# phymhan/supervised-gan

Hardware: AMD Instinct MI355X
Metric: train-step images/sec, fcgan 512x512 bs=1/GPU (higher is better)
Workload: dtype f32 (bf16x3 MFMA); 1 GPU; fcgan deconv-G(ngf32, z 8x8x8) + 3x PatchGAN-D(ndf32, n_layers 3, scale 1/2/4) 512x512 bs=1, n_update_D=1 n_update_G=2, Adam, pool 50 (BASELINE configs[1] shape, fp32 compute); synthetic batches resident in HBM (ring of 64); parallelism=dp1, global_batch=1, hip_graph=True, skip_wasted_D_wgrad=False

## Files before the change

### supervised-gan_amd/csrc/sgan_ew.hip

```cpp
#include "sgan_reduce.h"

thread_local char g_sgan_err[512] = {0};
thread_local const char* g_sgan_last_kernel = "";
thread_local char g_sgan_last_variant[96] = {0};

int sgan_fail(int code, const char* fmt, ...) {
    va_list ap;
    va_start(ap, fmt);
    vsnprintf(g_sgan_err, sizeof(g_sgan_err), fmt, ap);
    va_end(ap);
    return code;
}

extern "C" const char* sgan_version(void) { return "sgan_hip 0.2 (gfx950; fp32 MFMA 16x16x4 + split-bf16 MFMA 32x32x16)"; }
extern "C" const char* sgan_last_error(void) { return g_sgan_err; }
extern "C" const char* sgan_last_kernel(void) { return g_sgan_last_kernel; }
extern "C" const char* sgan_last_variant(void) { return g_sgan_last_variant; }
extern "C" int sgan_stat_replicas(void) { return SGAN_STAT_REPLICAS; }
extern "C" int sgan_set_device(int32_t device_id) {
    hipError_t e = hipSetDevice(device_id);
    if (e != hipSuccess) {
        (void)hipGetLastError();
        return sgan_fail(SGAN_ERR_HIP, "hipSetDevice(%d): %s", (int)device_id, hipGetErrorString(e));
    }
    return SGAN_OK;
}
extern "C" int sgan_stream_device(void* stream, int32_t* device_id) {
    if (!device_id) return sgan_fail(SGAN_ERR_INVALID, "null device_id");
    hipDevice_t dev;
    hipError_t e = hipStreamGetDevice((hipStream_t)stream, &dev);
    if (e != hipSuccess) {
        (void)hipGetLastError();
        return sgan_fail(SGAN_ERR_HIP, "hipStreamGetDevice: %s", hipGetErrorString(e));
    }
    *device_id = (int32_t)dev;
    return SGAN_OK;
}

#define SG_PROF_MAX 8192
static bool g_prof_on = false;
static int g_prof_n = 0;
static hipEvent_t g_prof_e0[SG_PROF_MAX], g_prof_e1[SG_PROF_MAX];
static const char* g_prof_name[SG_PROF_MAX];
static bool g_prof_open = false;

void sg_prof_begin(hipStream_t st) {
    if (!g_prof_on || g_prof_n >= SG_PROF_MAX) return;
    if (hipEventCreate(&g_prof_e0[g_prof_n]) != hipSuccess || hipEventCreate(&g_prof_e1[g_prof_n]) != hipSuccess) return;
    (void)hipEventRecord(g_prof_e0[g_prof_n], st);
    g_prof_open = true;
}

void sg_prof_end(hipStream_t st, const char* name) {
    if (!g_prof_open) return;
    (void)hipEventRecord(g_prof_e1[g_prof_n], st);
    g_prof_name[g_prof_n] = name;
    ++g_prof_n;
    g_prof_open = false;
}

extern "C" int sgan_profile_enable(int on) {
    for (int i = 0; i < g_prof_n; ++i) {
        (void)hipEventDestroy(g_prof_e0[i]);
        (void)hipEventDestroy(g_prof_e1[i]);
    }
    g_prof_n = 0;
    g_prof_on = on != 0;
    return SGAN_OK;
}

extern "C" int sgan_profile_count(void) { return g_prof_n; }

extern "C" int sgan_profile_mark(void* stream) {
    sg_prof_begin((hipStream_t)stream);
    sg_prof_end((hipStream_t)stream, "null");
    return SGAN_OK;
}

extern "C" int sgan_profile_read(int i, const char** name, float* ms) {
    if (i < 0 || i >= g_prof_n || !name || !ms) return sgan_fail(SGAN_ERR_INVALID, "bad profile record index");
    *name = g_prof_name[i];
    if (hipEventElapsedTime(ms, g_prof_e0[i], g_prof_e1[i]) != hipSuccess) return sgan_fail(SGAN_ERR_HIP, "hipEventElapsedTime failed");
    return SGAN_OK;
}

struct SgNormBwdJob {
    float* dy; const float* x; const double* sums; float* dgamma; float* dbeta; unsigned* amax;
    SgNorm xn;
    int32_t dy_ld, x_ld, npix, C, sums_sq, sums_rep, blocks;
};
struct SgNormBwdTable { SgNormBwdJob j[8]; };

__global__ __launch_bounds__(256) void sg_norm_bwd_apply_kernel(const SgNormBwdTable T) {
    sg_warm_kernargs<(int)sizeof(SgNormBwdTable)>();
    const SgNormBwdJob& J = T.j[blockIdx.y];
    if ((int)blockIdx.x >= J.blocks) return;
    const int C = J.C;
    extern __shared__ __attribute__((aligned(16))) char smem[];
    float* cA = reinterpret_cast<float*>(smem);
    float* cMean = cA + C;
    float* cRstd = cMean + C;
    float* cS1 = cRstd + C;
    float* cS2 = cS1 + C;
    const double invM = 1.0 / (double)J.npix;
    for (int c = threadIdx.x; c < C; c += 256) {
        float mean, rstd;
        sg_mean_rstd(J.xn, C, c, mean, rstd);
        const float g = J.xn.gamma ? J.xn.gamma[c] : 1.f;
        cA[c] = g * rstd;
        cMean[c] = mean;
        cRstd[c] = rstd;
        const double s1 = sg_stat_sum(J.sums, c, J.sums_rep), s2 = sg_stat_sum(J.sums, J.sums_sq + c, J.sums_rep);
        cS1[c] = (float)(s1 * invM);
        cS2[c] = (float)(s2 * invM);
        if (blockIdx.x == 0) {
            if (J.dgamma) atomicAdd(&J.dgamma[c], (float)s2);
            if (J.dbeta) atomicAdd(&J.dbeta[c], (float)s1);
        }
    }
    SG_SYNC();
    const int CQ = C >> 2;
    const int64_t total = (int64_t)J.npix * CQ;
    float* dy = J.dy;
    const float* x = J.x;
    const int64_t stride = (int64_t)J.blocks * 256;
    float amax = 0.f;
    for (int64_t e0 = (int64_t)blockIdx.x * 256 + threadIdx.x; e0 < total; e0 += 4 * stride) {
        f32x4 d[4], xv[4];
        int64_t od[4];
        int cc[4];
#pragma unroll
        for (int u = 0; u < 4; ++u) {
            const int64_t e = e0 + u * stride;
            const bool ok = e < total;
            const int p = ok ? (int)(e / CQ) : 0;
            cc[u] = ok ? (int)(e - (int64_t)p * CQ) * 4 : 0;
            od[u] = ok ? (int64_t)p * J.dy_ld + cc[u] : -1;
            d[u] = *reinterpret_cast<const f32x4*>(dy + (ok ? od[u] : 0));
            xv[u] = *reinterpret_cast<const f32x4*>(x + (ok ? (int64_t)p * J.x_ld + cc[u] : 0));
        }
#pragma unroll
        for (int u = 0; u < 4; ++u) {
            if (od[u] < 0) continue;
            const int c = cc[u];
#pragma unroll
            for (int j = 0; j < 4; ++j) {
                const float xhat = (xv[u][j] - cMean[c + j]) * cRstd[c + j];
                d[u][j] = cA[c + j] * (d[u][j] - cS1[c + j] - xhat * cS2[c + j]);
                amax = fmaxf(amax, fabsf(d[u][j]));
            }
            *reinterpret_cast<f32x4*>(dy + od[u]) = d[u];
        }
    }
    if (J.amax) {
        for (int o = 32; o > 0; o >>= 1) amax = fmaxf(amax, __shfl_xor(amax, o));
        SG_SYNC();
        if ((threadIdx.x & 63) == 0) cA[threadIdx.x >> 6] = amax;
        SG_SYNC();
        if (threadIdx.x == 0) {
            const unsigned mine = __builtin_bit_cast(unsigned, fmaxf(fmaxf(cA[0], cA[1]), fmaxf(cA[2], cA[3])));
            if (mine > __hip_atomic_load(J.amax, __ATOMIC_RELAXED, __HIP_MEMORY_SCOPE_AGENT)) atomicMax(J.amax, mine);
        }
    }
}

extern "C" int sgan_norm_bwd_apply_multi(const sgan_norm_bwd_job* jobs, int32_t n, void* stream) {
    SGAN_CHECK(jobs && n >= 1 && n <= 8, "1..8 jobs");
    SgNormBwdTable T;
    int maxb = 1, maxC = 4;
    for (int i = 0; i < n; ++i) {
        const sgan_norm_bwd_job& S = jobs[i];
        SGAN_CHECK(S.dy && S.x && S.x_norm && S.x_norm->stats && S.bwd_sums, "null argument in job %d", i);
        SGAN_CHECK((S.C & 3) == 0 && S.C > 0 && S.C <= 4096 && S.dy_ld >= S.C && S.x_ld >= S.C && (S.dy_ld & 3) == 0 &&
                       (S.x_ld & 3) == 0 && S.npix > 0, "bad dims in job %d", i);
        SgNormBwdJob& J = T.j[i];
        J.dy = S.dy; J.x = S.x; J.sums = S.bwd_sums; J.dgamma = S.dgamma; J.dbeta = S.dbeta;
        J.amax = reinterpret_cast<unsigned*>(S.amax_out);
        J.xn = sg_norm_from(S.x_norm);
        J.dy_ld = S.dy_ld; J.x_ld = S.x_ld; J.npix = S.npix; J.C = S.C;
        J.sums_sq = S.bwd_sums_sq_stride ? S.bwd_sums_sq_stride : S.C;
        J.sums_rep = S.bwd_sums_rep_stride;
        const int64_t total = (int64_t)S.npix * (S.C >> 2);
        static const int chunk = getenv("SGAN_NBA_CHUNK") ? atoi(getenv("SGAN_NBA_CHUNK")) : 4;
        int blocks = sg_cdiv(total, 256 * (chunk > 0 ? chunk : 4));
        if (blocks > 2048) blocks = 2048;
        if (blocks < 1) blocks = 1;
        J.blocks = blocks;
        if (blocks > maxb) maxb = blocks;
        if (S.C > maxC) maxC = S.C;
    }
    hipLaunchKernelGGL(sg_norm_bwd_apply_kernel, dim3(maxb, n), dim3(256), (size_t)5 * maxC * 4, (hipStream_t)stream, T);
    SGAN_LAUNCH_CHECK();
    g_sgan_last_kernel = "sg_norm_bwd_apply_kernel";
    return SGAN_OK;
}

extern "C" int sgan_norm_bwd_apply(float* dy, int32_t dy_ld, const float* x, int32_t x_ld, int32_t npix, int32_t C,
                                   const sgan_norm_desc* x_norm, const double* bwd_sums, int32_t bwd_sums_sq_stride,
                                   float* dgamma, float* dbeta, void* stream) {
    sgan_norm_bwd_job j = {dy, dy_ld, x, x_ld, npix, C, x_norm, bwd_sums, bwd_sums_sq_stride, dgamma, dbeta, 0, nullptr};
    return sgan_norm_bwd_apply_multi(&j, 1, stream);
}

__global__ __launch_bounds__(256) void sg_mean_rstd_probe_kernel(SgNorm n, int C, float* out) {
    for (int c = threadIdx.x; c < C; c += 256) {
        float mean, rstd;
        sg_mean_rstd(n, C, c, mean, rstd);
        out[2 * c] = mean;
        out[2 * c + 1] = rstd;
    }
}

extern "C" int sgan_norm_mean_rstd_probe(const sgan_norm_desc* d, int32_t C, float* out, void* stream) {
    SGAN_CHECK(d && d->stats && out && C > 0 && d->count > 0, "bad argument");
    hipLaunchKernelGGL(sg_mean_rstd_probe_kernel, dim3(1), dim3(256), 0, (hipStream_t)stream, sg_norm_from(d), C, out);
    SGAN_LAUNCH_CHECK();
    return SGAN_OK;
}

__global__ __launch_bounds__(256) void sg_norm_apply_fwd_kernel(const float* u, int u_ld, SgNorm un, const float* mask,
                                                                const float* noise, float sigma, float* t, int t_ld, int npix,
                                                                int C) {
    extern __shared__ __attribute__((aligned(16))) char smem[];
    float* cMean = reinterpret_cast<float*>(smem);
    float* cA = cMean + C;
    float* cB = cA + C;
    for (int c = threadIdx.x; c < C; c += 256) {
        float mean = 0.f, rstd = 1.f;
        if (un.stats) sg_mean_rstd(un, C, c, mean, rstd);
        cMean[c] = mean;
        cA[c] = (un.gamma ? un.gamma[c] : 1.f) * rstd;
        cB[c] = un.beta ? un.beta[c] : 0.f;
    }
    SG_SYNC();
    const int CQ = C >> 2;
    const int64_t total = (int64_t)npix * CQ;
    for (int64_t e = (int64_t)blockIdx.x * 256 + threadIdx.x; e < total; e += (int64_t)gridDim.x * 256) {
        const int p = (int)(e / CQ), c = (int)(e - (int64_t)p * CQ) * 4;
        const f32x4 x = *reinterpret_cast<const f32x4*>(u + (int64_t)p * u_ld + c);
        f32x4 m = (f32x4){1.f, 1.f, 1.f, 1.f}, nz = (f32x4){0.f, 0.f, 0.f, 0.f};
        if (mask) m = *reinterpret_cast<const f32x4*>(mask + (int64_t)p * C + c);
        if (noise) nz = *reinterpret_cast<const f32x4*>(noise + (int64_t)p * C + c);
        f32x4 o;
#pragma unroll
        for (int j = 0; j < 4; ++j) o[j] = ((x[j] - cMean[c + j]) * cA[c + j] + cB[c + j]) * m[j] + sigma * nz[j];
        *reinterpret_cast<f32x4*>(t + (int64_t)p * t_ld + c) = o;
    }
}

__global__ __launch_bounds__(256) void sg_norm_apply_bwd_sums_kernel(float* dt, int dt_ld, const float* mask, const float* u,
                                                                     int u_ld, SgNorm un, double* sums, int npix, int C) {
    extern __shared__ __attribute__((aligned(16))) char smem[];
    float* cMean = reinterpret_cast<float*>(smem);
    float* cRstd = cMean + C;
    float* red = cRstd + C;
    for (int c = threadIdx.x; c < C; c += 256) {
        float mean = 0.f, rstd = 1.f;
        if (un.stats) sg_mean_rstd(un, C, c, mean, rstd);
        cMean[c] = mean;
        cRstd[c] = rstd;
    }
    for (int i = threadIdx.x; i < 2 * C; i += 256) red[i] = 0.f;
    SG_SYNC();
    const int CQ = C >> 2;
    const int64_t total = (int64_t)npix * CQ;
    if (256 % CQ == 0) {
        const int c = (threadIdx.x % CQ) * 4;
        const f32x4 mean = *reinterpret_cast<const f32x4*>(cMean + c), rstd = *reinterpret_cast<const f32x4*>(cRstd + c);
        f32x4 s1 = (f32x4){0.f, 0.f, 0.f, 0.f}, s2 = s1;
        for (int64_t e = (int64_t)blockIdx.x * 256 + threadIdx.x; e < total; e += (int64_t)gridDim.x * 256) {
            const int64_t p = e / CQ;
            f32x4 d = *reinterpret_cast<const f32x4*>(dt + p * dt_ld + c);
            const f32x4 x = *reinterpret_cast<const f32x4*>(u + p * u_ld + c);
            if (mask) {
                d *= *reinterpret_cast<const f32x4*>(mask + p * C + c);
                *reinterpret_cast<f32x4*>(dt + p * dt_ld + c) = d;
            }
            s1 += d;
            s2 += d * ((x - mean) * rstd);
        }
#pragma unroll
        for (int j = 0; j < 4; ++j) {
            atomicAdd(&red[c + j], s1[j]);
            atomicAdd(&red[C + c + j], s2[j]);
        }
    } else {
        for (int64_t e = (int64_t)blockIdx.x * 256 + threadIdx.x; e < total; e += (int64_t)gridDim.x * 256) {
            const int p = (int)(e / CQ), c = (int)(e - (int64_t)p * CQ) * 4;
            f32x4 d = *reinterpret_cast<const f32x4*>(dt + (int64_t)p * dt_ld + c);
            const f32x4 x = *reinterpret_cast<const f32x4*>(u + (int64_t)p * u_ld + c);
            if (mask) {
                const f32x4 m = *reinterpret_cast<const f32x4*>(mask + (int64_t)p * C + c);
                d *= m;
                *reinterpret_cast<f32x4*>(dt + (int64_t)p * dt_ld + c) = d;
            }
#pragma unroll
            for (int j = 0; j < 4; ++j) {
                const float xhat = (x[j] - cMean[c + j]) * cRstd[c + j];
                atomicAdd(&red[c + j], d[j]);
                atomicAdd(&red[C + c + j], d[j] * xhat);
            }
        }
    }
    SG_SYNC();
    for (int c = threadIdx.x; c < C; c += 256) {
        atomicAdd(&sums[c], (double)red[c]);
        atomicAdd(&sums[C + c], (double)red[C + c]);
    }
}

extern "C" int sgan_norm_apply_fwd(const float* u, int32_t u_ld, const sgan_norm_desc* u_norm, const float* mask,
                                   const float* noise, float sigma, float* t, int32_t t_ld, int32_t npix, int32_t C, void* stream) {
    SGAN_CHECK(u && t && npix > 0 && C > 0 && (C & 3) == 0 && u_ld >= C && t_ld >= C && (u_ld & 3) == 0 && (t_ld & 3) == 0, "bad argument");
    const int64_t total = (int64_t)npix * (C >> 2);
    int blocks = sg_cdiv(total, 256 * 2);
    if (blocks > 2048) blocks = 2048;
    if (blocks < 1) blocks = 1;
    hipLaunchKernelGGL(sg_norm_apply_fwd_kernel, dim3(blocks), dim3(256), (size_t)3 * C * 4, (hipStream_t)stream, u, u_ld,
                       sg_norm_from(u_norm), mask, noise, sigma, t, t_ld, npix, C);
    SGAN_LAUNCH_CHECK();
    return SGAN_OK;
}

extern "C" int sgan_norm_apply_bwd_sums(float* dt, int32_t dt_ld, const float* mask, const float* u, int32_t u_ld,
                                        const sgan_norm_desc* u_norm, double* bwd_sums, int32_t npix, int32_t C, void* stream) {
    SGAN_CHECK(dt && u && bwd_sums && npix > 0 && C > 0 && (C & 3) == 0 && u_ld >= C && dt_ld >= C, "bad argument");
    const int64_t total = (int64_t)npix * (C >> 2);
    int blocks = sg_cdiv(total, 256 * 8);
    if (blocks > 512) blocks = 512;
    if (blocks < 1) blocks = 1;
    hipLaunchKernelGGL(sg_norm_apply_bwd_sums_kernel, dim3(blocks), dim3(256), (size_t)4 * C * 4, (hipStream_t)stream, dt, dt_ld,
                       mask, u, u_ld, sg_norm_from(u_norm), bwd_sums, npix, C);
    SGAN_LAUNCH_CHECK();
    return SGAN_OK;
}

__device__ __forceinline__ int sg_refl(int i, int n) { return i < 0 ? -i : (i >= n ? 2 * (n - 1) - i : i); }

__global__ __launch_bounds__(256) void sg_pad_reflect_fwd_kernel(const float* x, int x_ld, int H, int W, int C, SgNorm xn, const float* mask,
                                                                 int pad, float* out, int out_ld) {
    extern __shared__ __attribute__((aligned(16))) char smem[];
    float* cSc = reinterpret_cast<float*>(smem);
    float* cSh = cSc + C;
    for (int c = threadIdx.x; c < C; c += 256) {
        float sc = 1.f, sh = 0.f;
        if (xn.stats) {
            float mean, rstd;
            sg_mean_rstd(xn, C, c, mean, rstd);
            const float gm = xn.gamma ? xn.gamma[c] : 1.f, bt = xn.beta ? xn.beta[c] : 0.f;
            sc = gm * rstd;
            sh = bt - mean * sc;
        }
        cSc[c] = sc;
        cSh[c] = sh;
    }
    SG_SYNC();
    const int CQ = C >> 2, Wp = W + 2 * pad, Hp = H + 2 * pad;
    const int64_t total = (int64_t)Hp * Wp * CQ;
    for (int64_t e = (int64_t)blockIdx.x * 256 + threadIdx.x; e < total; e += (int64_t)gridDim.x * 256) {
        const int c = (int)(e % CQ) * 4;
        const int64_t pp = e / CQ;
        const int px = (int)(pp % Wp), py = (int)(pp / Wp);
        const int64_t src = (int64_t)sg_refl(py - pad, H) * W + sg_refl(px - pad, W);
        f32x4 v = *reinterpret_cast<const f32x4*>(x + src * x_ld + c);
#pragma unroll
        for (int j = 0; j < 4; ++j) v[j] = sg_act(v[j] * cSc[c + j] + cSh[c + j], xn.act, xn.slope);
        if (mask) v *= *reinterpret_cast<const f32x4*>(mask + src * C + c);
        *reinterpret_cast<f32x4*>(out + pp * out_ld + c) = v;
    }
}

extern "C" int sgan_pad_reflect_fwd(const float* x, int32_t x_ld, int32_t H, int32_t W, int32_t C, const sgan_norm_desc* x_norm,
                                    const float* mask, int32_t pad, float* out, int32_t out_ld, void* stream) {
    SGAN_CHECK(x && out && H > 0 && W > 0 && C > 0 && (C & 3) == 0 && (x_ld & 3) == 0 && (out_ld & 3) == 0 && x_ld >= C && out_ld >= C,
               "bad argument");
    SGAN_CHECK(pad >= 0 && pad < H && pad < W, "reflection padding must be smaller than the image");
    const int64_t total = (int64_t)(H + 2 * pad) * (W + 2 * pad) * (C >> 2);
    int blocks = sg_cdiv(total, 256 * 4);
    if (blocks > 2048) blocks = 2048;
    hipLaunchKernelGGL(sg_pad_reflect_fwd_kernel, dim3(blocks), dim3(256), (size_t)2 * C * 4, (hipStream_t)stream, x, x_ld, H, W, C,
                       sg_norm_from(x_norm), mask, pad, out, out_ld);
    SGAN_LAUNCH_CHECK();
    return SGAN_OK;
}

__global__ __launch_bounds__(256) void sg_pad_reflect_bwd_kernel(const float* dout, int dout_ld, int H, int W, int C, int pad, const float* x,
                                                                 int x_ld, SgNorm xn, const float* mask, float* din, int din_ld,
                                                                 double* sums, int sums_sq) {
    extern __shared__ __attribute__((aligned(16))) char smem[];
    float* cMean = reinterpret_cast<float*>(smem);
    float* cRstd = cMean + C;
    float* cG = cRstd + C;
    float* cB = cG + C;
    double* red = reinterpret_cast<double*>(cB + C);
    for (int c = threadIdx.x; c < C; c += 256) {
        float mean = 0.f, rstd = 1.f;
        if (xn.stats) sg_mean_rstd(xn, C, c, mean, rstd);
        cMean[c] = mean;
        cRstd[c] = rstd;
        cG[c] = (xn.stats && xn.gamma) ? xn.gamma[c] : 1.f;
        cB[c] = (xn.stats && xn.beta) ? xn.beta[c] : 0.f;
    }
    for (int i = threadIdx.x; i < 2 * C; i += 256) red[i] = 0.0;
    SG_SYNC();
    const int CQ = C >> 2, Wp = W + 2 * pad;
    const int64_t total = (int64_t)H * W * CQ;
    const bool has_x = x != nullptr;
    for (int64_t e = (int64_t)blockIdx.x * 256 + threadIdx.x; e < total; e += (int64_t)gridDim.x * 256) {
        const int c = (int)(e % CQ) * 4;
        const int64_t pix = e / CQ;
        const int xx = (int)(pix % W), yy = (int)(pix / W);
        int ys[3], xs[3], ny = 0, nx = 0;
        ys[ny++] = yy + pad;
        if (yy >= 1 && yy <= pad) ys[ny++] = pad - yy;
        if (yy <= H - 2 && yy >= H - 1 - pad) ys[ny++] = pad + 2 * (H - 1) - yy;
        xs[nx++] = xx + pad;
        if (xx >= 1 && xx <= pad) xs[nx++] = pad - xx;
        if (xx <= W - 2 && xx >= W - 1 - pad) xs[nx++] = pad + 2 * (W - 1) - xx;
        f32x4 d = (f32x4){0.f, 0.f, 0.f, 0.f};
        for (int a = 0; a < ny; ++a)
            for (int b = 0; b < nx; ++b) d += *reinterpret_cast<const f32x4*>(dout + ((int64_t)ys[a] * Wp + xs[b]) * dout_ld + c);
        if (mask) d *= *reinterpret_cast<const f32x4*>(mask + pix * C + c);
        if (has_x) {
            const f32x4 xv = *reinterpret_cast<const f32x4*>(x + pix * x_ld + c);
#pragma unroll
            for (int j = 0; j < 4; ++j) {
                const float xhat = (xv[j] - cMean[c + j]) * cRstd[c + j];
                const float y = xn.stats ? cG[c + j] * xhat + cB[c + j] : xv[j];
                d[j] *= sg_act_grad(y, xn.act, xn.slope);
                if (sums) {
                    atomicAdd(&red[c + j], (double)d[j]);
                    atomicAdd(&red[C + c + j], (double)(d[j] * xhat));
                }
            }
        }
        *reinterpret_cast<f32x4*>(din + pix * din_ld + c) = d;
    }
    if (sums) {
        SG_SYNC();
        for (int c = threadIdx.x; c < C; c += 256) {
            atomicAdd(&sums[c], red[c]);
            atomicAdd(&sums[(sums_sq ? sums_sq : C) + c], red[C + c]);
        }
    }
}

extern "C" int sgan_pad_reflect_bwd(const float* dout, int32_t dout_ld, int32_t H, int32_t W, int32_t C, int32_t pad, const float* x,
                                    int32_t x_ld, const sgan_norm_desc* x_norm, const float* mask, float* din, int32_t din_ld,
                                    double* bwd_sums, int32_t bwd_sums_sq_stride, void* stream) {
    SGAN_CHECK(dout && din && H > 0 && W > 0 && C > 0 && (C & 3) == 0 && (dout_ld & 3) == 0 && (din_ld & 3) == 0 && dout_ld >= C && din_ld >= C,
               "bad argument");
    SGAN_CHECK(pad >= 0 && 2 * pad < H && 2 * pad < W, "reflection padding must be smaller than half the image");
    SGAN_CHECK(!(bwd_sums && !x), "bwd_sums needs x");
    SGAN_CHECK(!x || ((x_ld & 3) == 0 && x_ld >= C), "bad x_ld");
    const int64_t total = (int64_t)H * W * (C >> 2);
    int blocks = sg_cdiv(total, 256 * 4);
    if (blocks > 1024) blocks = 1024;
    hipLaunchKernelGGL(sg_pad_reflect_bwd_kernel, dim3(blocks), dim3(256), (size_t)4 * C * 4 + (size_t)2 * C * 8, (hipStream_t)stream, dout,
                       dout_ld, H, W, C, pad, x, x_ld, sg_norm_from(x ? x_norm : nullptr), mask, din, din_ld, bwd_sums, bwd_sums_sq_stride);
    SGAN_LAUNCH_CHECK();
    return SGAN_OK;
}

#define SG_IMGLOSS_BLOCKS 256
__device__ __forceinline__ void sg_block_partial(double acc, double* part) {
    __shared__ double wsum[4];
    const double sum = sg_block_sum<4>(acc, wsum);
    if (threadIdx.x == 0) part[blockIdx.x] = sum;
}

__global__ __launch_bounds__(64) void sg_imgloss_fin_kernel(const double* part, int nparts, double scale, float* loss_out) {
    double acc = 0.0;
    for (int i = threadIdx.x; i < nparts; i += 64) acc += part[i];
    acc = sg_wave_sum(acc);
    if (threadIdx.x == 0) loss_out[0] = (float)(acc * scale);
}

__global__ __launch_bounds__(256) void sg_l1w_fwd_kernel(const float* x, int x_ld, const float* y, int y_ld, int npix, int C,
                                                         const float* a, int a_ld, const float* wts, int nw, float lambda,
                                                         double* part, float* g, int g_ld) {
    const double inv = 1.0 / ((double)npix * (double)C);
    double acc = 0.0;
    for (int p = blockIdx.x * 256 + threadIdx.x; p < npix; p += gridDim.x * 256) {
        float w = 1.f;
        if (a) {
            if (nw == 0) w = a[(int64_t)p * a_ld];
            for (int i = 0; i < nw; ++i) w += (a[(int64_t)p * a_ld + i] + 1.f) * 0.5f * (wts[i] - 1.f);
        }
        for (int c = 0; c < g_ld; ++c) {
            float gv = 0.f;
            if (c < C) {
                const float d = x[(int64_t)p * x_ld + c] - y[(int64_t)p * y_ld + c];
                acc += (double)(fabsf(d) * w);
                gv = (d > 0.f ? 1.f : (d < 0.f ? -1.f : 0.f)) * w * lambda * (float)inv;
// ... 1829 lines not shown
```

Before: 543.3 images/sec.

## Flatten multi-job norm backward apply grid and overlap first loads with stat setup

Replaces the 2D (maxb x jobs) launch of the normalization-backward apply kernel with a flat 1D grid where each job gets only its own block range, found by a prefix table. The per-block chunk count is sized against CU count times an assumed residency so the grid roughly fills the GPU once, and blocks grid-stride over their job. The first batch of dy/x loads is issued before the per-channel mean/rstd/stat shared-memory setup, which hides setup latency. The old path is kept behind an env var and for very large jobs. Fewer blocks means per-channel setup is repeated less often, but each block does more serial work.

Result: no change. 545.2 images/sec, median of 3 (+0.3%).

```diff
diff --git a/supervised-gan_amd/csrc/sgan_ew.hip b/supervised-gan_amd/csrc/sgan_ew.hip
--- a/supervised-gan_amd/csrc/sgan_ew.hip
+++ b/supervised-gan_amd/csrc/sgan_ew.hip
@@ -89,10 +89,9 @@
     SgNorm xn;
     int32_t dy_ld, x_ld, npix, C, sums_sq, sums_rep, blocks;
 };
-struct SgNormBwdTable { SgNormBwdJob j[8]; };
-
-__global__ __launch_bounds__(256) void sg_norm_bwd_apply_kernel(const SgNormBwdTable T) {
-    sg_warm_kernargs<(int)sizeof(SgNormBwdTable)>();
+struct SgNormBwdTable { int32_t first[9]; int32_t n; SgNormBwdJob j[8]; };
+
+__device__ __forceinline__ void sg_norm_bwd_apply_legacy(const SgNormBwdTable& T) {
     const SgNormBwdJob& J = T.j[blockIdx.y];
     if ((int)blockIdx.x >= J.blocks) return;
     const int C = J.C;
@@ -164,10 +163,129 @@
     }
 }
 
+__device__ __forceinline__ void sg_norm_bwd_apply_flat(const SgNormBwdTable& T) {
+    int i = 0;
+#pragma unroll
+    for (int k = 1; k < 8; ++k)
+        if ((int)blockIdx.x >= T.first[k]) i = k;
+    const SgNormBwdJob& J = T.j[i];
+    const int b = (int)blockIdx.x - T.first[i];
+    const int C = J.C, CQ = C >> 2;
+    const int total = J.npix * CQ;
+    const int stride = J.blocks * 256;
+    const int sp = stride / CQ, sq = stride - sp * CQ;
+    float* dy = J.dy;
+    const float* x = J.x;
+    const int64_t lastd = (int64_t)(J.npix - 1) * J.dy_ld + C - 4, lastx = (int64_t)(J.npix - 1) * J.x_ld + C - 4;
+    int e = b * 256 + (int)threadIdx.x;
+    int p = e / CQ, q = e - p * CQ;
+    f32x4 d[4], xv[4];
+    int64_t od[4];
+    int cc[4];
+    extern __shared__ __attribute__((aligned(16))) char smem[];
+    float* cA = reinterpret_cast<float*>(smem);
+    float* cMean = cA + C;
+    float* cRstd = cMean + C;
+    float* cS1 = cRstd + C;
+    float* cS2 = cS1 + C;
+    float amax = 0.f;
+    for (bool first = true;; first = false) {
+#pragma unroll
+        for (int u = 0; u < 4; ++u) {
+            const bool ok = e < total;
+            cc[u] = q * 4;
+            const int64_t offd = (int64_t)p * J.dy_ld + cc[u], offx = (int64_t)p * J.x_ld + cc[u];
+            od[u] = ok ? offd : -1;
+            d[u] = *reinterpret_cast<const f32x4*>(dy + (offd < lastd ? offd : lastd));
+            xv[u] = *reinterpret_cast<const f32x4*>(x + (offx < lastx ? offx : lastx));
+            e += stride; p += sp; q += sq;
+            if (q >= CQ) { q -= CQ; ++p; }
+        }
+        if (first) {
+            const double invM = 1.0 / (double)J.npix;
+            for (int c = threadIdx.x; c < C; c += 256) {
+                float mean, rstd;
+                sg_mean_rstd(J.xn, C, c, mean, rstd);
+                const float g = J.xn.gamma ? J.xn.gamma[c] : 1.f;
+                cA[c] = g * rstd;
+                cMean[c] = mean;
+                cRstd[c] = rstd;
+                const double s1 = sg_stat_sum(J.sums, c, J.sums_rep), s2 = sg_stat_sum(J.sums, J.sums_sq + c, J.sums_rep);
+                cS1[c] = (float)(s1 * invM);
+                cS2[c] = (float)(s2 * invM);
+                if (b == 0) {
+                    if (J.dgamma) atomicAdd(&J.dgamma[c], (float)s2);
+                    if (J.dbeta) atomicAdd(&J.dbeta[c], (float)s1);
+                }
+            }
+            SG_SYNC();
+        }
+#pragma unroll
+        for (int u = 0; u < 4; ++u) {
+            if (od[u] < 0) continue;
+            const int c = cc[u];
+#pragma unroll
+            for (int j = 0; j < 4; ++j) {
+                const float xhat = (xv[u][j] - cMean[c + j]) * cRstd[c + j];
+                d[u][j] = cA[c + j] * (d[u][j] - cS1[c + j] - xhat * cS2[c + j]);
+                amax = fmaxf(amax, fabsf(d[u][j]));
+            }
+            *reinterpret_cast<f32x4*>(dy + od[u]) = d[u];
+        }
+        if (e >= total) break;
+    }
+    if (J.amax) {
+        for (int o = 32; o > 0; o >>= 1) amax = fmaxf(amax, __shfl_xor(amax, o));
+        SG_SYNC();
+        if ((threadIdx.x & 63) == 0) cA[threadIdx.x >> 6] = amax;
+        SG_SYNC();
+        if (threadIdx.x == 0) {
+            const unsigned mine = __builtin_bit_cast(unsigned, fmaxf(fmaxf(cA[0], cA[1]), fmaxf(cA[2], cA[3])));
+            if (mine > __hip_atomic_load(J.amax, __ATOMIC_RELAXED, __HIP_MEMORY_SCOPE_AGENT)) atomicMax(J.amax, mine);
+        }
+    }
+}
+
+__global__ __launch_bounds__(256) void sg_norm_bwd_apply_kernel(const SgNormBwdTable T) {
+    sg_warm_kernargs<(int)sizeof(SgNormBwdTable)>();
+    if (T.n)
+        sg_norm_bwd_apply_flat(T);
+    else
+        sg_norm_bwd_apply_legacy(T);
+}
+
+#define SG_NBA_RESIDENT 5
+#define SG_NBA_MIN_CHUNKS 4
+static int sg_nba_cus() {
+    static int cus = 0;
+    if (cus == 0) {
+        int dev = 0, n = 0;
+        if (hipGetDevice(&dev) != hipSuccess || hipDeviceGetAttribute(&n, hipDeviceAttributeMultiprocessorCount, dev) != hipSuccess || n < 1)
+            n = 256;
+        cus = n;
+    }
+    return cus;
+}
+
 extern "C" int sgan_norm_bwd_apply_multi(const sgan_norm_bwd_job* jobs, int32_t n, void* stream) {
     SGAN_CHECK(jobs && n >= 1 && n <= 8, "1..8 jobs");
+    static const bool legacy_env = getenv("SGAN_NBA_LEGACY") && atoi(getenv("SGAN_NBA_LEGACY")) != 0;
+    static const int chunk = getenv("SGAN_NBA_CHUNK") ? atoi(getenv("SGAN_NBA_CHUNK")) : 0;
     SgNormBwdTable T;
     int maxb = 1, maxC = 4;
+    int64_t sum = 0;
+    bool legacy = legacy_env;
+    for (int i = 0; i < n; ++i) {
+        const int64_t total = (int64_t)jobs[i].npix * (jobs[i].C >> 2);
+        sum += total;
+        if (total > (1ll << 28)) legacy = true;
+    }
+    int per = chunk > 0 ? chunk : SG_NBA_MIN_CHUNKS;
+    if (!legacy && chunk <= 0) {
+        const int64_t fill = sg_cdiv(sum, (int64_t)256 * SG_NBA_RESIDENT * sg_nba_cus());
+        if (fill > per) per = (int)((fill + 3) / 4 * 4);
+    }
+    int nwg = 0;
     for (int i = 0; i < n; ++i) {
         const sgan_norm_bwd_job& S = jobs[i];
         SGAN_CHECK(S.dy && S.x && S.x_norm && S.x_norm->stats && S.bwd_sums, "null argument in job %d", i);
@@ -181,15 +299,18 @@
         J.sums_sq = S.bwd_sums_sq_stride ? S.bwd_sums_sq_stride : S.C;
         J.sums_rep = S.bwd_sums_rep_stride;
         const int64_t total = (int64_t)S.npix * (S.C >> 2);
-        static const int chunk = getenv("SGAN_NBA_CHUNK") ? atoi(getenv("SGAN_NBA_CHUNK")) : 4;
-        int blocks = sg_cdiv(total, 256 * (chunk > 0 ? chunk : 4));
-        if (blocks > 2048) blocks = 2048;
+        int blocks = sg_cdiv(total, (int64_t)256 * per);
+        if (legacy && blocks > 2048) blocks = 2048;
         if (blocks < 1) blocks = 1;
         J.blocks = blocks;
+        T.first[i] = nwg;
+        nwg += blocks;
         if (blocks > maxb) maxb = blocks;
         if (S.C > maxC) maxC = S.C;
     }
-    hipLaunchKernelGGL(sg_norm_bwd_apply_kernel, dim3(maxb, n), dim3(256), (size_t)5 * maxC * 4, (hipStream_t)stream, T);
+    for (int i = n; i < 9; ++i) T.first[i] = INT32_MAX;
+    T.n = legacy ? 0 : n;
+    hipLaunchKernelGGL(sg_norm_bwd_apply_kernel, legacy ? dim3(maxb, n) : dim3(nwg), dim3(256), (size_t)5 * maxC * 4, (hipStream_t)stream, T);
     SGAN_LAUNCH_CHECK();
     g_sgan_last_kernel = "sg_norm_bwd_apply_kernel";
     return SGAN_OK;
```
